# tsnb66/afivo-streamer

Hardware: AMD Instinct MI355X
Metric: cell-updates/s (fluid+MG V-cycle) (higher is better)
Workload: dtype f64; 1 GPU; s1-64; n_cell=64, leaf_cells=134217728, boxes=585, levels=4, coarse_solve=exact separable, fused_rhs=interior, face_field=from phi in the flux, vcycle_graphs=False, parallelism=single-gpu

## Files before the change

afivo-streamer_amd/csrc/afh_mg.hip:

```cpp
#include <hip/hip_ext.h>

#include <algorithm>
#include <cfloat>
#include <cmath>
#include <map>
#include <type_traits>

#include "afh_internal.h"
#include "afh_cs_direct.h"
#include "afh_pfmg_dev.h"

#include <mutex>

namespace afh {

struct Coef {
  double c[7];
};

constexpr int MAXMG = 16;
constexpr int CS_BOTTOM_SWEEPS = 16;
constexpr int CS_SMALL_CELLS = 4096;
constexpr int CS_DS_N = 16;
constexpr int CS_DS_CELLS = 1024;
// ... 866 lines not shown
__device__ __forceinline__ double apply7(const double *x, size_t c, size_t sj,
                                         size_t sk, const Coef &cf) {
  return cf.c[0] * x[c] + cf.c[1] * x[c - 1] + cf.c[2] * x[c + 1] +
         cf.c[3] * x[c - sj] + cf.c[4] * x[c + sj] + cf.c[5] * x[c - sk] +
         cf.c[6] * x[c + sk];
}

struct StConst {
  Coef cf;
  __device__ double apply(int, size_t, const double *x, size_t c, size_t sj, size_t sk) const {
    return apply7(x, c, sj, sk, cf);
  }
};

struct StVar {
  const double *const *vp, *const *bp;
  __device__ double apply(int id, size_t cv, const double *x, size_t c, size_t sj,
                          size_t sk) const {
    const double *v = vp[id - 1] + 7 * cv, *b = bp[id - 1];
    double a = v[0] * x[c] + v[1] * x[c - 1] + v[2] * x[c + 1] + v[3] * x[c - sj] +
               v[4] * x[c + sj] + v[5] * x[c - sk] + v[6] * x[c + sk];
    if (b) a = a - b[cv];
    return a;
  }
};

template <bool MAX, int K, bool GRAD = false>
__global__ void __launch_bounds__(256)
    k_residual(const double *__restrict__ phi, const double *__restrict__ rhs,
               double *__restrict__ tmp, const int32_t *__restrict__ ids,
               int nc, size_t bsz, Coef cf0, unsigned long long *red,
               const Coef *__restrict__ cft = nullptr,
               const afh_box_meta *__restrict__ meta = nullptr,
               double *__restrict__ nrm = nullptr, double gfac = 0.0) {
  const int t = blockIdx.x * blockDim.x + threadIdx.x;
  double mx = 0.0;
  if (t < nc * nc * (nc / K)) {
    const int id = ids[blockIdx.y];
    const Coef cf = cft ? cft[meta[id - 1].lvl - 1] : cf0;
    int i, j, kq;
    cell3(t, nc, i, j, kq);
    const int ng = nc + 2;
    const size_t sj = ng, sk = (size_t)ng * ng;
    const size_t o = (size_t)(id - 1) * bsz, c0 = ix3(ng, i, j, (kq - 1) * K + 1);
    const double *x = phi + o;
    double z[K + 2], xm[K], xp[K], ym[K], yp[K], r[K];
#pragma unroll
    for (int q = 0; q < K + 2; q++) z[q] = x[c0 + (q - 1) * sk];
#pragma unroll
    for (int q = 0; q < K; q++) {
      const size_t c = c0 + q * sk;
      xm[q] = x[c - 1];
      xp[q] = x[c + 1];
      ym[q] = x[c - sj];
      yp[q] = x[c + sj];
      r[q] = rhs[o + c];
    }
#pragma unroll
    for (int q = 0; q < K; q++) {
      const double a = cf.c[0] * z[q + 1] + cf.c[1] * xm[q] + cf.c[2] * xp[q] +
                       cf.c[3] * ym[q] + cf.c[4] * yp[q] + cf.c[5] * z[q] +
                       cf.c[6] * z[q + 2];
      const double v = r[q] - a;
      st_nt<AFH_NT_MG>(tmp + (o + c0 + q * sk), v);
      mx = fmax(mx, fabs(v));
    }
    if constexpr (GRAD) {
      const afh_box_meta &mb = meta[id - 1];
      const double gx = gfac / mb.dr[0], gy = gfac / mb.dr[1], gz = gfac / mb.dr[2];
#pragma unroll
      for (int q = 0; q < K; q++) {
        const double pv = z[q + 1];
        const double fxl = gx * (pv - xm[q]), fxh = gx * (xp[q] - pv);
        const double fyl = gy * (pv - ym[q]), fyh = gy * (yp[q] - pv);
        const double fzl = gz * (pv - z[q]), fzh = gz * (z[q + 2] - pv);
        const double a = fxl + fxh, b = fyl + fyh, c = fzl + fzh;
        st_nt<AFH_NT_MG>(nrm + (o + c0 + q * sk), 0.5 * sqrt(a * a + b * b + c * c));
      }
    }
  }
  if (MAX) block_max_to_shard(mx, red);
}

template <class St>
__global__ void k_rstr_fas(double *__restrict__ phi,
                           const double *__restrict__ rhs,
                           double *__restrict__ tmp,
                           const afh_box_meta *__restrict__ meta,
                           const int32_t *__restrict__ ids, int nc, size_t bsz,
                           St st) {
  const int hn = nc >> 1;
  const int t = blockIdx.x * blockDim.x + threadIdx.x;
  if (t >= hn * hn * hn) return;
  const int id = ids[blockIdx.y];
  const afh_box_meta &m = meta[id - 1];
  int i, j, k;
  cell3(t, hn, i, j, k);
  const int ng = nc + 2;
  const size_t sj = ng, sk = (size_t)ng * ng;
  const size_t o = (size_t)(id - 1) * bsz;
  const double *x = phi + o, *r = rhs + o;
  const int fi = 2 * i - 1, fj = 2 * j - 1, fk = 2 * k - 1;
  double sr = 0.0, sp = 0.0;
#pragma unroll
  for (int q = 0; q < 8; q++) {
    const int ci = fi + (q & 1), cj = fj + ((q >> 1) & 1), ck = fk + (q >> 2);
    const size_t c = ix3(ng, ci, cj, ck);
    const size_t cv = ((size_t)(ck - 1) * nc + (cj - 1)) * nc + (ci - 1);
    const double res = r[c] - st.apply(id, cv, x, c, sj, sk);
    if (q == 0) {
      sr = res;
      sp = x[c];
    } else {
      sr += res;
      sp += x[c];
    }
  }
  const size_t po = (size_t)(m.parent - 1) * bsz +
                    ix3(ng, ((m.ix[0] - 1) & 1) * hn + i,
                        ((m.ix[1] - 1) & 1) * hn + j,
                        ((m.ix[2] - 1) & 1) * hn + k);
  tmp[po] = 0.125 * sr;
  phi[po] = 0.125 * sp;
}

template <int K>
__global__ void __launch_bounds__(256)
    k_rstr_fas_col(double *__restrict__ phi, const double *__restrict__ rhs,
                   double *__restrict__ tmp, const afh_box_meta *__restrict__ meta,
                   const int32_t *__restrict__ ids, int nc, size_t bsz, Coef cf,
                   const double *__restrict__ fine) {
  const int hn = nc >> 1;
  const int t = blockIdx.x * blockDim.x + threadIdx.x;
  if (t >= hn * hn * (hn / K)) return;
  const int id = ids[blockIdx.y];
  const afh_box_meta &m = meta[id - 1];
  int i, j, kq;
  cell3(t, hn, i, j, kq);
  const int k0 = (kq - 1) * K + 1;
  const int ng = nc + 2;
  const size_t sj = ng;
  const size_t o = (size_t)(id - 1) * bsz;
  const double *x = fine + o, *r = rhs + o;
  const int fi = 2 * i - 1, fj = 2 * j - 1, f0 = 2 * k0 - 1;
  double c[2 * K + 2][4];
#pragma unroll
  for (int p = 0; p < 2 * K + 2; p++) {
    const size_t b = ix3(ng, fi, fj, f0 - 1 + p);
    c[p][0] = x[b];
    c[p][1] = x[b + 1];
    c[p][2] = x[b + sj];
    c[p][3] = x[b + sj + 1];
  }
  const size_t pb = (size_t)(m.parent - 1) * bsz;
  const int pi = ((m.ix[0] - 1) & 1) * hn + i, pj = ((m.ix[1] - 1) & 1) * hn + j,
            pk = ((m.ix[2] - 1) & 1) * hn;
#pragma unroll
  for (int q = 0; q < K; q++) {
    double sr = 0.0, sp = 0.0;
#pragma unroll
    for (int h = 0; h < 2; h++) {
      const int p = 2 * q + 1 + h;
      const size_t b = ix3(ng, fi, fj, f0 - 1 + p);
      const double xm0 = x[b - 1], xp0 = x[b + 2];
      const double xm1 = x[b + sj - 1], xp1 = x[b + sj + 2];
      const double ym0 = x[b - sj], ym1 = x[b - sj + 1];
// ... 241 lines not shown
    if (dd[3] < 1 && !later(3)) f[fx(1, i, j + 1, k)] = iy * (bc - pc) / dd[3];
    if (dd[4] < 1 && !later(4)) f[fx(2, i, j, k)] = iz * (pc - bc) / dd[4];
    if (dd[5] < 1 && !later(5)) f[fx(2, i, j, k + 1)] = iz * (bc - pc) / dd[5];
  }
}

__global__ void k_field_norm(const double *__restrict__ fcv,
                             double *__restrict__ nrm,
                             const int32_t *__restrict__ ids, int nc, size_t bsz,
                             size_t fsz) {
  const int t = blockIdx.x * blockDim.x + threadIdx.x;
  if (t >= nc * nc * nc) return;
  const int id = ids[blockIdx.y];
  int i, j, k;
  cell3(t, nc, i, j, k);
  const int nf = nc + 1;
  const size_t d3 = (size_t)nf * nf * nf;
  const double *f = fcv + (size_t)(id - 1) * fsz;
  const size_t fb = ((size_t)(k - 1) * nf + (j - 1)) * nf + (i - 1);
  const double a = f[fb] + f[fb + 1], b = f[d3 + fb] + f[d3 + fb + nf],
               cc = f[2 * d3 + fb] + f[2 * d3 + fb + (size_t)nf * nf];
  nrm[(size_t)(id - 1) * bsz + ix3(nc + 2, i, j, k)] = 0.5 * sqrt(a * a + b * b + cc * cc);
}

__global__ void k_corr_tmp(const double *__restrict__ phi,
                           double *__restrict__ tmp,
                           const int32_t *__restrict__ ids, size_t bsz) {
  const size_t t = (size_t)blockIdx.x * blockDim.x + threadIdx.x;
  if (t >= bsz) return;
  const size_t o = (size_t)(ids[blockIdx.y] - 1) * bsz + t;
  tmp[o] = phi[o] - tmp[o];
}

__global__ void k_box_copy(const double *__restrict__ src,
                           double *__restrict__ dst,
                           const int32_t *__restrict__ ids, size_t bsz) {
  const size_t t = (size_t)blockIdx.x * blockDim.x + threadIdx.x;
  if (t >= bsz) return;
  const size_t o = (size_t)(ids[blockIdx.y] - 1) * bsz + t;
  dst[o] = src ? src[o] : 0.0;
}

template <int K>
__global__ void __launch_bounds__(256)
    k_prolong(double *__restrict__ phi, const double *__restrict__ tmp,
              const afh_box_meta *__restrict__ meta,
              const int32_t *__restrict__ ids, int nc, size_t bsz) {
  const int t = blockIdx.x * blockDim.x + threadIdx.x;
  if (t >= nc * nc * (nc / K)) return;
  const int id = ids[blockIdx.y];
  const afh_box_meta &m = meta[id - 1];
  int i, j, kq;
  cell3(t, nc, i, j, kq);
  const int k0 = (kq - 1) * K + 1;
  const int ng = nc + 2, hn = nc >> 1;
  const size_t sk = (size_t)ng * ng;
  const int o0 = ((m.ix[0] - 1) & 1) * hn, o1 = ((m.ix[1] - 1) & 1) * hn,
            o2 = ((m.ix[2] - 1) & 1) * hn;
  const int i1 = o0 + ((i + 1) >> 1), i2 = i1 + 1 - 2 * (i & 1);
  const int j1 = o1 + ((j + 1) >> 1), j2 = j1 + 1 - 2 * (j & 1);
  const int P = o2 + ((k0 + 1) >> 1);
  const double *p = tmp + (size_t)(m.parent - 1) * bsz;
  const size_t c = (size_t)(id - 1) * bsz + ix3(ng, i, j, k0);
  double pv[K / 2 + 2][4], ph[K];
#pragma unroll
  for (int q = 0; q < K / 2 + 2; q++) {
    const size_t b = ix3(ng, 0, 0, P - 1 + q);
    pv[q][0] = p[b + (size_t)j1 * ng + i1];
    pv[q][1] = p[b + (size_t)j1 * ng + i2];
    pv[q][2] = p[b + (size_t)j2 * ng + i1];
    pv[q][3] = p[b + (size_t)j2 * ng + i2];
  }
#pragma unroll
  for (int q = 0; q < K; q++) ph[q] = phi[c + q * sk];
#pragma unroll
  for (int q = 0; q < K; q++) {
    const int a = (q & 1) ? (q + 1) / 2 : q / 2 + 1;
    const int b = (q & 1) ? (q + 3) / 2 : q / 2;
    st_nt<AFH_NT_MG>(phi + (c + q * sk),
                     ph[q] + (27 / 64.0) * pv[a][0] + (9 / 64.0) * pv[a][1] +
                         (9 / 64.0) * pv[a][2] + (3 / 64.0) * pv[a][3] +
                         (9 / 64.0) * pv[b][0] + (3 / 64.0) * pv[b][1] +
                         (3 / 64.0) * pv[b][2] + (1 / 64.0) * pv[b][3]);
  }
}

__global__ void k_gradient(const double *__restrict__ phi,
                           double *__restrict__ fcv, double *__restrict__ nrm,
                           const afh_box_meta *__restrict__ meta,
                           const int32_t *__restrict__ ids, int nc, size_t bsz,
                           size_t fsz, double fac) {
  const int t = blockIdx.x * blockDim.x + threadIdx.x;
  if (t >= nc * nc * nc) return;
  const int id = ids[blockIdx.y];
  const afh_box_meta &m = meta[id - 1];
  const int i = t % nc + 1, j = (t / nc) % nc + 1, k = t / (nc * nc) + 1;
  const int ng = nc + 2, nf = nc + 1;
  const double *p = phi + (size_t)(id - 1) * bsz;
  double *f = fcv ? fcv + (size_t)(id - 1) * fsz : nullptr;
  const size_t c = ix3(ng, i, j, k), sj = ng, sk = (size_t)ng * ng;
  const double ix_ = fac / m.dr[0], iy = fac / m.dr[1], iz = fac / m.dr[2];
  const double fxl = ix_ * (p[c] - p[c - 1]), fxh = ix_ * (p[c + 1] - p[c]);
  const double fyl = iy * (p[c] - p[c - sj]), fyh = iy * (p[c + sj] - p[c]);
  const double fzl = iz * (p[c] - p[c - sk]), fzh = iz * (p[c + sk] - p[c]);
  const size_t d3 = (size_t)nf * nf * nf;
  auto fx = [&](int d, int a, int b, int cc) {
    return (size_t)d * d3 + ((size_t)(cc - 1) * nf + (b - 1)) * nf + (a - 1);
  };
  if (fcv) {
    f[fx(0, i, j, k)] = fxl;
    if (i == nc) f[fx(0, nc + 1, j, k)] = fxh;
    f[fx(1, i, j, k)] = fyl;
    if (j == nc) f[fx(1, i, nc + 1, k)] = fyh;
    f[fx(2, i, j, k)] = fzl;
    if (k == nc) f[fx(2, i, j, nc + 1)] = fzh;
  }
  if (nrm) {
    const double a = fxl + fxh, b = fyl + fyh, cc = fzl + fzh;
    nrm[(size_t)(id - 1) * bsz + c] = 0.5 * sqrt(a * a + b * b + cc * cc);
  }
}

template <int NC, int K, bool NT = false, bool FC = true>
__global__ void __launch_bounds__(256)
    k_gradient_t(const double *__restrict__ phi, double *__restrict__ fcv,
                 double *__restrict__ nrm, const int32_t *__restrict__ ids,
                 size_t bsz, size_t fsz, const afh_box_meta *__restrict__ meta,
                 double fac) {
  constexpr int R = 256 / NC < NC ? 256 / NC : NC;
  constexpr int NG = NC + 2, NF = NC + 1;
  constexpr size_t SJ = NG, SK = (size_t)NG * NG, D3 = (size_t)NF * NF * NF;
  const Blk B = xcd_block();
  const int i = threadIdx.x % NC + 1;
  const int j = (B.x % (NC / R)) * R + threadIdx.x / NC + 1;
  const int k0 = (B.x / (NC / R)) * K + 1;
  const int id = ids[B.y];
  const double ix_ = fac / meta[id - 1].dr[0], iy = fac / meta[id - 1].dr[1],
               iz = fac / meta[id - 1].dr[2];
  const double *p = phi + (size_t)(id - 1) * bsz;
  double *f = fcv + (size_t)(id - 1) * fsz;
  double *nb = nrm ? nrm + (size_t)(id - 1) * bsz : nullptr;
  const size_t c0 = ((size_t)k0 * NG + j) * NG + i;
  double pc[K + 2], xm[K], xp[K], ym[K], yp[K];
#pragma unroll
  for (int q = 0; q < K + 2; q++) pc[q] = p[c0 + (q - 1) * SK];
#pragma unroll
  for (int q = 0; q < K; q++) {
    const size_t c = c0 + q * SK;
    xm[q] = p[c - 1];
    xp[q] = p[c + 1];
    ym[q] = p[c - SJ];
    yp[q] = p[c + SJ];
  }
#pragma unroll
  for (int q = 0; q < K; q++) {
    const int k = k0 + q;
    const double pv = pc[q + 1];
    const double fxl = ix_ * (pv - xm[q]), fxh = ix_ * (xp[q] - pv);
    const double fyl = iy * (pv - ym[q]), fyh = iy * (yp[q] - pv);
    const double fzl = iz * (pv - pc[q]), fzh = iz * (pc[q + 2] - pv);
    const size_t fb = ((size_t)(k - 1) * NF + (j - 1)) * NF + (i - 1);
    if (FC) {
      st_nt<NT>(f + fb, fxl);
      if (i == NC) st_nt<NT>(f + fb + 1, fxh);
      st_nt<NT>(f + D3 + fb, fyl);
      if (j == NC) st_nt<NT>(f + D3 + fb + NF, fyh);
// ... 731 lines not shown
    for (int nb = 0; nb < 6; nb++)
      if ((fm >> nb) & 1) rv = rv + b2r[(size_t)nb * L0.np + p] * B.bc[nb].value;
    if (vbc[q]) rv = rv + vbc[q][e];
    b[p] = rv;
    X0[p] = phi[c];
  }
  __syncthreads();
  PF_T(10);
  int cur = 0;
  const int iters = afh_pf::pf_solve_block(Lg, nl, wave_from, A, Aw, soff, Pw, X0, X1, b, r,
                                           &slot, tol, max_iter, &cur);
  const double *x = cur ? X1 : X0;
  for (int u = threadIdx.x; u < nid * n3; u += blockDim.x) {
    const int q = u / n3, e = u % n3, id = ids[q];
    const afh_box_meta &m = meta[id - 1];
    const int i = e % nc + 1, j = (e / nc) % nc + 1, k = e / (nc * nc) + 1;
    (void)q;
    const int p = (((m.ix[2] - 1) * nc + k - 1) * ny + (m.ix[1] - 1) * nc + j - 1) * nx +
                  (m.ix[0] - 1) * nc + i - 1;
    phi[(size_t)(id - 1) * bsz + ix3(nc + 2, i, j, k)] = x[p];
  }
  if (threadIdx.x == 0 && iters_out) *iters_out = iters;
#ifdef AFH_PFMG_TIMING
  PF_T(11);
  if (threadIdx.x == 0) {
    const unsigned long long *a = afh_pf::pf_tacc();
    printf("PFTIME nt %d np %d nl %d wave %d iters %d wall10ns %llu | relax %llu/%llu res %llu/%llu "
           "rstr %llu/%llu interp %llu/%llu dot %llu/%llu handoff %llu | wave relax %llu/%llu "
           "res %llu/%llu rstr %llu/%llu interp %llu/%llu | gather %llu scatter %llu\n",
           (int)blockDim.x, np, nl, wave_from, iters, wall_clock64() - w0, a[0], a[12], a[1],
           a[13], a[2], a[14], a[3], a[15], a[4], a[16], a[5], a[6], a[18], a[7], a[19], a[8],
           a[20], a[9], a[21], a[10], a[11]);
  }
#endif
}

}

using namespace afh;

#ifndef AFH_RES_K
#define AFH_RES_K 0
#endif
#ifndef AFH_RSTR_K
#define AFH_RSTR_K 4
#endif
struct afh_mg {
  afh_tree *t = nullptr;
  afh_mg_desc d;
  std::vector<Coef> lvl_c;
  CsParams P;
  int small_from = 0;
  size_t small_lds = 0;
  double *d_dtab = nullptr;
  std::vector<double> h_dtab;
  int tab_bc[6] = {0, 0, 0, 0, 0, 0};
  int fused_min = 0;
  bool force_tiles = false;
  bool rccl_capture = false;
  std::vector<char> rhs_halo;
  int vc_max_lvl = 0;
  bool grad_nt = true;
  uint64_t phi_gc_gen = UINT64_MAX;
  uint64_t phi_gc_meth = UINT64_MAX;
  int *cs_iters = nullptr;
  bool cs_direct_small = true;
  int cs_ds_cells = CS_DS_CELLS;
  bool pair_push = true;
  bool prolong_push = true;
  bool rstr_push = true;
  bool in_fmg = false;
  bool pair_xfetch = true;
  int tiles_min = 256;
  int *d_cycles = nullptr;
  int cycles_host = 0;
  bool cycles_on_dev = false;
  double *d_norm = nullptr;
  Coef *d_lvl_c = nullptr;
  std::vector<double> h_norm;
  bool rstr_col = true;
  int rstr_k = AFH_RSTR_K;
  int res_k = AFH_RES_K;
  int prolong_k = 4;
  int rstr_bs = 256;
  int wave_cells = CS_WAVE_CELLS;
  double *d_q[3] = {nullptr, nullptr, nullptr}, *d_qt[3] = {nullptr, nullptr, nullptr};
  double *d_e[3] = {nullptr, nullptr, nullptr};
  double *w1 = nullptr, *w2 = nullptr;
  int q_bc[6] = {0, 0, 0, 0, 0, 0};
  double *alt = nullptr;
  double *alt_priv = nullptr;
  std::vector<double *> h_vp, h_bp, h_dd, h_bv;
  std::vector<int32_t *> h_ix;
  std::vector<int> h_lsf_n;
  double **d_vp = nullptr, **d_bp = nullptr, **d_dd = nullptr, **d_bv = nullptr;
  int32_t **d_ix = nullptr;
  int *d_lsf_n = nullptr;
  int i_lsf = 0;
  bool var_dirty = false, any_var = false, any_lsf = false;
  struct Graph {
    hipGraphExec_t exec = nullptr;
    uint64_t meth_gen = 0;
    bool warm = false;
    std::vector<hipGraphExec_t> segs;
    std::vector<std::array<int32_t, 4>> ops;
    bool eager_only = false;
    void release() {
      if (exec) hipGraphExecDestroy(exec);
      for (hipGraphExec_t s : segs)
        if (s) hipGraphExecDestroy(s);
      exec = nullptr;
      segs.clear();
      ops.clear();
    }
  };
  std::map<int, Graph> graphs;
  bool use_graphs = true;
  bool seg_graphs = true;
  int64_t n_replays = 0, n_seg_replays = 0;
  std::vector<char> lvl_var;
  LevelList ids_c, ids_v, leaves_c, leaves_v, parents_c, parents_v, lsf_leaves;
  double *cs_old = nullptr;
  bool csd_on = true, csd_ok = false;
  std::vector<double> h_v1;
  int h_v1_id = 0;
  uint64_t v1_gen = 1, csd_v_gen = 0, csd_meth_gen = UINT64_MAX;
  double *d_csd_ainv = nullptr, *d_csd_g = nullptr;
  int grad_iv = 0;
  double grad_fac = -1.0;
  uint64_t grad_phi_gen = UINT64_MAX, grad_norm_gen = UINT64_MAX;
  std::map<int, std::vector<double>> h_vl1;
  std::vector<double> pf_a7;
  uint64_t pf_v1_gen = 0, pf_meth_gen = UINT64_MAX;
  int pf_nl = 0, pf_np = 0, pf_lds = 0, pf_wave = 0;
  bool pf_stage = false;
  PfLvl *d_pf_lvl = nullptr;
  double *d_pf_A = nullptr, *d_pf_P = nullptr, *d_pf_b2r = nullptr, *d_pf_x = nullptr;
  uint8_t *d_pf_fmask = nullptr;
  const double **d_pf_vbc = nullptr;
};

static int32_t build_table(afh_mg *mg) {
  const afh_bc *bc = mg->t->meth[mg->d.i_phi].bc;
  CsParams &P = mg->P;
  mg->h_dtab.assign((size_t)MAXMG * 64 * 2, 0.0);
  for (int m = 0; m < P.n_mg; m++)
    for (int c = 0; c < 64; c++) {
      double d = P.cdiag[m];
      for (int nb = 1; nb <= 6; nb++) {
        const int dd = (nb - 1) >> 1;
        const bool low = ((nb - 1) & 1) == 0;
        const int at = low ? (c >> (2 * dd)) & 1 : (c >> (2 * dd + 1)) & 1;
        if (!at || P.per[dd]) continue;
        if (bc[nb - 1].type == AFH_BC_DIRICHLET) d = d - P.hc[m][dd];
        else d = d + P.hc[m][dd];
      }
      mg->h_dtab[(m * 64 + c) * 2] = d;
      mg->h_dtab[(m * 64 + c) * 2 + 1] = 1 / d;
    }
  for (int q = 0; q < 6; q++) mg->tab_bc[q] = bc[q].type;
  AFH_HIP(hipStreamSynchronize(mg->t->stream));
  AFH_HIP(hipMemcpy(mg->d_dtab, mg->h_dtab.data(),
                    mg->h_dtab.size() * sizeof(double), hipMemcpyHostToDevice));
  P.dtab = mg->d_dtab;
  return AFH_OK;
}
// ... 100 lines not shown
  mg->h_ix.assign(t->nb, nullptr), mg->h_lsf_n.assign(t->nb, 0);
  mg->lvl_c.resize(t->nlvl);
  for (int l = 1; l <= t->nlvl; l++) {
    const double *dr = &t->lvl_dr[3 * (l - 1)];
    Coef &c = mg->lvl_c[l - 1];
    for (int q = 0; q < 3; q++) {
      double inv = 1 / (dr[q] * dr[q]);
      c.c[1 + 2 * q] = inv;
      c.c[2 + 2 * q] = inv;
    }
    double s = c.c[1];
    for (int q = 2; q < 7; q++) s = s + c.c[q];
    c.c[0] = -s - d->helmholtz_lambda;
  }
  AFH_HIP(hipMalloc(&mg->d_lvl_c, sizeof(Coef) * t->nlvl));
  AFH_HIP(hipMemcpy(mg->d_lvl_c, mg->lvl_c.data(), sizeof(Coef) * t->nlvl,
                    hipMemcpyHostToDevice));
  CsParams &P = mg->P;
  memset(&P, 0, sizeof P);
  int m = 0;
  for (int q = 0; q < 3; q++) {
    P.dims[0][q] = t->cgs[q];
    P.hc[0][q] = mg->lvl_c[0].c[1 + 2 * q];
  }
  P.cdiag[0] = mg->lvl_c[0].c[0];
  P.cmask = 63;
  for (int q = 0; q < 3; q++) {
    P.per[q] = t->periodic[q];
    if (P.per[q]) P.cmask &= ~(3 << (2 * q));
  }
  for (;;) {
    int *n = P.dims[m];
    bool ok = (n[0] % 2 == 0) && (n[1] % 2 == 0) && (n[2] % 2 == 0) &&
              n[0] >= 4 && n[1] >= 4 && n[2] >= 4 && m < MAXMG - 1;
    for (int q = 0; q < 3; q++) ok = ok && !(P.per[q] && (n[q] / 2) % 2 != 0);
    if (!ok) break;
    for (int q = 0; q < 3; q++) {
      P.dims[m + 1][q] = n[q] / 2;
      P.hc[m + 1][q] = 0.25 * P.hc[m][q];
    }
    const double *h = P.hc[m + 1];
    P.cdiag[m + 1] = -(h[0] + h[0] + h[1] + h[1] + h[2] + h[2]) -
                     d->helmholtz_lambda;
    m++;
  }
  P.n_mg = m + 1;
  mg->small_from = P.n_mg - 1;
  while (mg->small_from > 0) {
    const int *n = P.dims[mg->small_from - 1];
    if ((long)n[0] * n[1] * n[2] > CS_SMALL_CELLS) break;
    mg->small_from--;
  }
  mg->small_lds = 0;
  for (int q = 0; q < P.n_mg; q++) {
    P.halo[q] = 1;
    const int nx = P.dims[q][0], ny = P.dims[q][1];
    const bool p2 = nx > 0 && ny > 0 && (nx & (nx - 1)) == 0 && (ny & (ny - 1)) == 0;
    P.lg[q] = p2 ? (__builtin_ctz(nx) | (__builtin_ctz(ny) << 8)) : -1;
    if (q >= mg->small_from)
      mg->small_lds += 2 * sizeof(double) * (size_t)P.dims[q][0] * P.dims[q][1] *
                       P.dims[q][2];
  }
  if (mg->small_lds + sizeof(CsParams) + MAXMG * 128 * sizeof(double) > 160 * 1024)
    return set_error(AFH_ERR_UNSUPPORTED, "coarse-solver LDS levels too large");
  AFH_HIP(raise_dyn_lds((const void *)k_cs_small, (int)mg->small_lds));
  AFH_HIP(hipMalloc(&mg->d_dtab, (size_t)MAXMG * 64 * 2 * sizeof(double)));
  if (int32_t e = build_table(mg)) return e;
  if (const char *env = getenv("AFH_RCCL_CAPTURE")) mg->rccl_capture = atoi(env) != 0;
  if (const char *env = getenv("AFH_GSRB_FUSED_MIN_BOXES"))
    mg->fused_min = atoi(env);
  else if (fused_nc_ok(t->nc))
    mg->fused_min = t->nc >= 32 ? 64 : 1;
  if (const char *env = getenv("AFH_GSRB_TILES")) mg->force_tiles = atoi(env) != 0;
  if (const char *env = getenv("AFH_GRAPHS")) mg->use_graphs = atoi(env) != 0;
  if (const char *env = getenv("AFH_RSTR_COL")) mg->rstr_col = atoi(env) != 0;
  if (const char *env = getenv("AFH_RSTR_K")) {
    const int k = atoi(env);
    mg->rstr_k = k == 8 ? 8 : k == 4 ? 4 : 2;
  }
  if (const char *env = getenv("AFH_RES_K"))
    mg->res_k = atoi(env) == 8 ? 8 : atoi(env) == 2 ? 2 : 4;
  if (const char *env = getenv("AFH_PROLONG_K"))
    mg->prolong_k = atoi(env) == 8 ? 8 : atoi(env) == 2 ? 2 : 4;
  if (const char *env = getenv("AFH_CS_ELEC_DIRECT")) mg->csd_on = atoi(env) != 0;
  if (const char *env = getenv("AFH_CS_DIRECT_SMALL")) mg->cs_direct_small = atoi(env) != 0;
  if (const char *env = getenv("AFH_GSRB_TILES_MIN")) mg->tiles_min = atoi(env);
  if (const char *env = getenv("AFH_PAIR_XFETCH")) mg->pair_xfetch = atoi(env) != 0;
  if (const char *env = getenv("AFH_PAIR_PUSH")) mg->pair_push = atoi(env) != 0;
  if (const char *env = getenv("AFH_PROLONG_PUSH")) mg->prolong_push = atoi(env) != 0;
  if (const char *env = getenv("AFH_RSTR_PUSH")) mg->rstr_push = atoi(env) != 0;
  AFH_HIP(hipMalloc(&mg->cs_iters, sizeof(int)));
  AFH_HIP(hipMalloc(&mg->d_cycles, sizeof(int)));
  if (fused_nc_ok(t->nc) && mg->fused_min > 0) {
    bool any = false;
    for (int l = 2; l <= t->nlvl; l++) any |= t->lvl_total[l - 1] >= mg->fused_min;
    if (any) {
      if (!t->alt) {
        if (int32_t e2 = pool_alloc((void **)&t->alt_base,
                                    (size_t)t->nb * t->bsz * sizeof(double), "alt"))
          return e2;
        t->alt = t->alt_base;
        AFH_HIP(hipMemsetAsync(t->alt, 0, (size_t)t->nb * t->bsz * sizeof(double),
                               t->stream));
      }
      t->alt_refs++;
      mg->alt = t->alt;
    }
  }
  for (int q = 0; q < P.n_mg; q++) {
    size_t n = (size_t)(P.dims[q][0] + 2) * (P.dims[q][1] + 2) * (P.dims[q][2] + 2);
    AFH_HIP(hipMalloc(&P.u[q], n * sizeof(double)));
    AFH_HIP(hipMalloc(&P.f[q], n * sizeof(double)));
    AFH_HIP(hipMemsetAsync(P.u[q], 0, n * sizeof(double), t->stream));
    AFH_HIP(hipMemsetAsync(P.f[q], 0, n * sizeof(double), t->stream));
  }
  if (d->coarse_mode == AFH_COARSE_DIRECT) {
    const size_t n = (size_t)P.dims[0][0] * P.dims[0][1] * P.dims[0][2];
    for (int q = 0; q < 3; q++) {
      const size_t nd = P.dims[0][q];
      AFH_HIP(hipMalloc(&mg->d_q[q], nd * nd * sizeof(double)));
      AFH_HIP(hipMalloc(&mg->d_qt[q], nd * nd * sizeof(double)));
      AFH_HIP(hipMalloc(&mg->d_e[q], nd * sizeof(double)));
    }
    AFH_HIP(hipMalloc(&mg->w1, n * sizeof(double)));
    AFH_HIP(hipMalloc(&mg->w2, n * sizeof(double)));
    if (int32_t e = build_direct(mg)) return e;
  }
  AFH_HIP(hipStreamSynchronize(t->stream));
  *out = mg;
  return AFH_OK;
}

int32_t afh_mg_destroy(afh_mg *mg) {
  if (!mg) return AFH_OK;
  hipStreamSynchronize(mg->t->stream);
  for (auto &g : mg->graphs) g.second.release();
  for (int q = 0; q < mg->P.n_mg; q++) {
    hipFree(mg->P.u[q]);
    hipFree(mg->P.f[q]);
  }
  hipFree(mg->d_dtab);
  for (int q = 0; q < 3; q++) hipFree(mg->d_q[q]), hipFree(mg->d_qt[q]), hipFree(mg->d_e[q]);
  hipFree(mg->w1);
  hipFree(mg->w2);
  hipFree(mg->d_csd_ainv), hipFree(mg->d_csd_g);
  hipFree(mg->d_pf_lvl), hipFree(mg->d_pf_A), hipFree(mg->d_pf_P), hipFree(mg->d_pf_b2r);
  hipFree(mg->d_pf_x), hipFree(mg->d_pf_fmask), hipFree((void *)mg->d_pf_vbc);
  hipFree(mg->alt_priv);
  if (mg->alt && --mg->t->alt_refs == 0) {
    hipFree(mg->t->alt_base);
    mg->t->alt = mg->t->alt_base = nullptr;
  }
  for (auto *v : {&mg->h_vp, &mg->h_bp, &mg->h_dd, &mg->h_bv})
    for (double *q : *v) hipFree(q);
  for (int32_t *q : mg->h_ix) hipFree(q);
  hipFree(mg->d_vp), hipFree(mg->d_bp), hipFree(mg->d_dd), hipFree(mg->d_bv);
  hipFree(mg->d_ix), hipFree(mg->d_lsf_n), hipFree(mg->cs_old);
  hipFree(mg->cs_iters);
  hipFree(mg->d_cycles);
  hipFree(mg->d_norm);
  hipFree(mg->d_lvl_c);
  for (LevelList *L : {&mg->ids_c, &mg->ids_v, &mg->leaves_c, &mg->leaves_v,
                       &mg->parents_c, &mg->parents_v, &mg->lsf_leaves})
    hipFree(L->d);
  delete mg;
  return AFH_OK;
// ... 220 lines not shown

static bool rstr_push(const afh_mg *mg, int lvl, bool ghosts_valid) {
  const int nc = mg->t->nc;
  return ghosts_valid && mg->rstr_push && pair_push(mg) && !mg->any_var &&
         (nc == 4 || nc == 8 || nc == 16) && fused_level(mg, lvl - 1);
}

static int32_t update_coarse(afh_mg *mg, int lvl, bool ghosts_valid = false) {
  afh_tree *t = mg->t;
  const int nc = t->nc, hn = nc / 2;
  double *phi = t->ccv(mg->d.i_phi), *rhs = t->ccv(mg->d.i_rhs), *tmp = t->ccv(mg->d.i_tmp);
  if (rstr_push(mg, lvl, ghosts_valid)) {
    const GcArgs ga = t->gc_args(mg->d.i_phi);
    const int nid = t->ids.n(lvl), np = t->parents.n(lvl - 1);
    if (nid) {
      with_size<4, 8, 16>(nc, [&](auto NC_) {
        constexpr int NC = decltype(NC_)::value;
        hipLaunchKernelGGL(k_rstr_box<NC>, dim3(nid), dim3(NC >= 16 ? 512 : 64), 0, t->stream,
                           phi, rhs, tmp, t->d_boxes, t->ids.at(lvl), t->bsz,
                           mg->lvl_c[lvl - 1], ga);
      });
      AFH_LAUNCH_CHECK("k_rstr_box");
    }
    if (np) {
      with_bool(nc == 16, [&](auto big) {
        constexpr int NT = decltype(big)::value ? 512 : 256;
        hipLaunchKernelGGL(k_parent_rhs_box<NT>, dim3(np), dim3(NT), 0, t->stream, phi, rhs,
                           tmp, t->d_boxes, t->parents.at(lvl - 1), nc, t->bsz,
                           mg->lvl_c[lvl - 2]);
      });
      AFH_LAUNCH_CHECK("k_parent_rhs_box");
    }
    return AFH_OK;
  }
  const int RK = mg->rstr_k, BS = mg->rstr_bs;
  const int kc = !mg->rstr_col               ? 0
                 : RK == 8 && hn % 8 == 0    ? 8
                 : RK >= 4 && hn % 4 == 0    ? 4
                 : hn % 2 == 0               ? 2
                                             : 0;
  auto rstr = [&](const LevelList &L, auto st) -> int32_t {
    const int nid = L.n(lvl);
    if (!nid) return AFH_OK;
    bool col = false;
    if constexpr (!is_var<decltype(st)>)
      col = with_col(kc, [&](auto K_) {
        constexpr int K = decltype(K_)::value;
        hipLaunchKernelGGL(k_rstr_fas_col<K>, dim3((hn * hn * (hn / K) + BS - 1) / BS, nid),
                           dim3(BS), 0, t->stream, phi, rhs, tmp, t->d_boxes, L.at(lvl), nc,
                           t->bsz, st.cf, phi);
      });
    if (!col)
      hipLaunchKernelGGL(k_rstr_fas<decltype(st)>, dim3((hn * hn * hn + 255) / 256, nid),
                         dim3(256), 0, t->stream, phi, rhs, tmp, t->d_boxes, L.at(lvl), nc,
                         t->bsz, st);
    AFH_LAUNCH_CHECK(is_var<decltype(st)> ? "k_rstr_fas_v" : "k_rstr_fas");
    return AFH_OK;
  };
  int32_t e;
  if ((e = const_then_var(mg, lvl, t->ids, mg->ids_c, mg->ids_v, rstr))) return e;
  if ((e = call_hook(t, AFH_HOOK_RESTRICT, lvl, mg->d.i_phi)) ||
      (e = call_hook(t, AFH_HOOK_RESTRICT, lvl, mg->d.i_tmp)))
    return e;
  if ((e = gc_lvl(t, lvl - 1, mg->d.i_phi, 1, fused_level(mg, lvl - 1),
                  fused_level(mg, lvl - 1) ? 2 : 1)))
    return e;
  auto parent_rhs = [&](const LevelList &P, auto st) -> int32_t {
    const int np = P.n(lvl - 1);
    if (!np) return AFH_OK;
    hipLaunchKernelGGL(k_parent_rhs<decltype(st)>, dim3((unsigned)((t->bsz + 255) / 256), np),
                       dim3(256), 0, t->stream, phi, rhs, tmp, P.at(lvl - 1), nc, t->bsz, st);
    AFH_LAUNCH_CHECK(is_var<decltype(st)> ? "k_parent_rhs_v" : "k_parent_rhs");
    return AFH_OK;
  };
  return const_then_var(mg, lvl - 1, t->parents, mg->parents_c, mg->parents_v, parent_rhs);
}

static bool prolong_push(const afh_mg *mg, int lvl) {
  const int nc = mg->t->nc;
  return mg->prolong_push && pair_push(mg) && (nc == 4 || nc == 8 || nc == 16) &&
         fused_level(mg, lvl);
}

static int32_t correct_children(afh_mg *mg, int lvl) {
  afh_tree *t = mg->t;
  const int np = t->parents.n(lvl - 1), nc = t->nc;
  if (np) {
    hipLaunchKernelGGL(k_corr_tmp, dim3((unsigned)((t->bsz + 255) / 256), np),
                       dim3(256), 0, t->stream, t->ccv(mg->d.i_phi),
                       t->ccv(mg->d.i_tmp), t->parents.at(lvl - 1), t->bsz);
    AFH_LAUNCH_CHECK("k_corr_tmp");
  }
  const int nid = t->ids.n(lvl);
  if (nid && prolong_push(mg, lvl)) {
    const GcArgs ga = t->gc_args(mg->d.i_phi);
    with_size<4, 8, 16>(nc, [&](auto NC_) {
      constexpr int NC = decltype(NC_)::value;
      hipLaunchKernelGGL(k_prolong_box<NC>, dim3(nid), dim3(RbBox<NC>::NT), 0, t->stream,
                         t->ccv(mg->d.i_phi), t->ccv(mg->d.i_tmp), t->d_boxes, t->ids.at(lvl),
                         t->bsz, ga);
    });
    AFH_LAUNCH_CHECK("k_prolong_box");
  } else if (nid) {
    double *fphi = t->ccv(mg->d.i_phi);
    const int want = mg->prolong_k;
    const int K = want == 8 && nc % 8 == 0 ? 8 : want >= 4 && nc % 4 == 0 ? 4 : 2;
    const dim3 grid((nc * nc * (nc / K) + 255) / 256, nid);
    with_col(K, [&](auto K_) {
      hipLaunchKernelGGL(k_prolong<decltype(K_)::value>, grid, dim3(256), 0, t->stream, fphi,
                         t->ccv(mg->d.i_tmp), t->d_boxes, t->ids.at(lvl), nc, t->bsz);
    });
    AFH_LAUNCH_CHECK("k_prolong");
  }
  return AFH_OK;
}

extern "C++" {
template <int NC>
__global__ void __launch_bounds__(1024)
    k_cs_electrode(double *__restrict__ x, double *__restrict__ r,
                   const double *__restrict__ v, const double *__restrict__ b,
                   GcArgs ga, double dr0, double dr1, double dr2,
                   int *__restrict__ iters) {
  constexpr int NG = NC + 2, N3 = NC * NC * NC, G3 = NG * NG * NG;
  constexpr int SJ = NG, SK = NG * NG;
  __shared__ double X[G3], R[N3];
  __shared__ double s_d[16], s_m[16];
  const int tid = threadIdx.x, nt = blockDim.x;
  for (int e = tid; e < G3; e += nt) X[e] = x[e];
  for (int e = tid; e < N3; e += nt) {
    const int i = e % NC + 1, j = (e / NC) % NC + 1, k = e / (NC * NC) + 1;
    R[e] = r[ix3(NG, i, j, k)];
  }
  __syncthreads();
  constexpr int CPT = (N3 + 1023) / 1024;
  double old[CPT];
  int it;
  for (it = 1; it <= 200000; it++) {
#pragma unroll
    for (int q = 0; q < CPT; q++) {
      const int e = tid + q * nt;
      if (e < N3) {
        const int i = e % NC + 1, j = (e / NC) % NC + 1, k = e / (NC * NC) + 1;
        old[q] = X[ix3(NG, i, j, k)];
      }
    }
    for (int n = 1; n <= 2; n++) {
      for (int e = tid; e < N3; e += nt) {
        const int i = e % NC + 1, j = (e / NC) % NC + 1, k = e / (NC * NC) + 1;
        const int c = ix3(NG, i, j, k);
        const double *w = v + 7 * (size_t)e;
        double r1 = R[e];
        if (b) r1 = r1 + b[e];
        if (((i + j + k + n) & 1) == 0)
          X[c] = (r1 - w[1] * X[c - 1] - w[2] * X[c + 1] - w[3] * X[c - SJ] -
                  w[4] * X[c + SJ] - w[5] * X[c - SK] - w[6] * X[c + SK]) /
                 w[0];
        if (b) R[e] = r1 - b[e];
      }
      __syncthreads();
      for (int e = tid; e < 6 * NC * NC; e += nt) {
        const int nb = e / (NC * NC) + 1, ab = e % (NC * NC);
        const int d = (nb - 1) >> 1;
        const bool low = ((nb - 1) & 1) == 0;
        const int ta = d == 0 ? 1 : 0, tb = d == 2 ? 1 : 2;
        int p[3], q1[3];
        p[ta] = ab % NC + 1;
        p[tb] = ab / NC + 1;
        p[d] = low ? 0 : NC + 1;
        q1[0] = p[0], q1[1] = p[1], q1[2] = p[2];
        q1[d] = low ? 1 : NC;
        const afh_bc bc = ga.bc[nb - 1];
        const double drd = d == 0 ? dr0 : d == 1 ? dr1 : dr2;
        double c0, c1;
        switch (bc.type) {
        case AFH_BC_DIRICHLET: c0 = 2; c1 = -1; break;
        case AFH_BC_NEUMANN: c0 = drd * (low ? -1 : 1); c1 = 1; break;
        default: c0 = 1; c1 = 0; break;
        }
        X[ix3(NG, p[0], p[1], p[2])] = c0 * bc.value + c1 * X[ix3(NG, q1[0], q1[1], q1[2])];
      }
      __syncthreads();
    }
    double dm = 0.0, mm = 0.0;
#pragma unroll
    for (int q = 0; q < CPT; q++) {
      const int e = tid + q * nt;
      if (e < N3) {
        const int i = e % NC + 1, j = (e / NC) % NC + 1, k = e / (NC * NC) + 1;
        const double pv = X[ix3(NG, i, j, k)];
        dm = fmax(dm, fabs(pv - old[q]));
        mm = fmax(mm, fabs(pv));
      }
    }
    for (int o = 32; o > 0; o >>= 1) {
// ... 426 lines not shown
                               t->stream, P, m, n);
      }
      done = cyc + 1;
      if (tol) {
        double rr;
        if (int32_t e = norm2(1, rr)) return e;
        if (rr / bb < eps) break;
      }
    }
    AFH_LAUNCH_CHECK("coarse solver cycle");
    mg->cycles_host = done, mg->cycles_on_dev = false;
  }
  hipLaunchKernelGGL(k_cs_scatter, dim3((n3 + 255) / 256, nid), dim3(256), 0,
                     t->stream, P, t->ccv(mg->d.i_phi), t->d_boxes,
                     t->ids.at(1), nc, t->bsz);
  AFH_LAUNCH_CHECK("k_cs_scatter");
  return gc_lvl(t, 1, mg->d.i_phi, 1);
}

static int32_t box_copy(afh_tree *t, int lvl, const double *src, double *dst) {
  const int n = t->ids.n(lvl);
  if (!n) return AFH_OK;
  hipLaunchKernelGGL(k_box_copy, dim3((unsigned)((t->bsz + 255) / 256), n),
                     dim3(256), 0, t->stream, src, dst, t->ids.at(lvl), t->bsz);
  AFH_LAUNCH_CHECK("k_box_copy");
  return AFH_OK;
}

int32_t afh_mg_fas_fmg(afh_mg *mg, int32_t set_residual, int32_t have_guess) {
  if (!mg) return set_error(AFH_ERR_ARG, "null mg");
  afh_tree *t = mg->t;
  AFH_LIVE(t, "afh_mg_fas_fmg");
  if (int32_t ebc = phi_bc_check(mg)) return ebc;
  t->touch(mg->d.i_phi), t->touch(mg->d.i_rhs), t->touch(mg->d.i_tmp);
  const int nl = t->nlvl, i_phi = mg->d.i_phi;
  double *phi = t->ccv(i_phi), *tmp = t->ccv(mg->d.i_tmp);
  int32_t e;
  if ((e = prepare_all(mg))) return e;
  if (have_guess) {
    for (int lvl = nl; lvl >= 2; lvl--) {
      if (lvl == nl && (e = gc_lvl(t, lvl, i_phi, 1, fused_level(mg, lvl)))) return e;
      if ((e = update_coarse(mg, lvl))) return e;
    }
  } else {
    for (int lvl = nl; lvl >= 2; lvl--) {
      if ((e = box_copy(t, lvl, nullptr, phi)) ||
          (e = restrict_boxes(t, t->ids.at(lvl), t->ids.n(lvl), mg->d.i_rhs)) ||
          (e = call_hook(t, AFH_HOOK_RESTRICT, lvl, mg->d.i_rhs)))
        return e;
    }
  }
  if ((e = box_copy(t, 1, phi, tmp)) ||
      (e = afh_mg_fas_vcycle(mg, set_residual && nl == 1, 1)))
    return e;
  for (int lvl = 2; lvl <= nl; lvl++) {
    if ((e = box_copy(t, lvl, phi, tmp)) || (e = correct_children(mg, lvl)) ||
        (e = gc_lvl(t, lvl, i_phi, 1, fused_level(mg, lvl))))
      return e;
    mg->phi_gc_gen = t->gen[i_phi];
    mg->phi_gc_meth = t->meth_gen;
    mg->in_fmg = true;
    e = afh_mg_fas_vcycle(mg, set_residual && lvl == nl, lvl);
    mg->in_fmg = false;
    if (e) return e;
  }
  return AFH_OK;
}

}

static bool grad_fused(const afh_mg *mg, int max_lvl) {
  return mg->grad_iv > 0 && !mg->any_var && max_lvl == mg->t->nlvl;
}

static int32_t residual_levels(afh_mg *mg, int max_lvl, bool max_out) {
  afh_tree *t = mg->t;
  const int nc = t->nc, n3 = nc * nc * nc;
  auto *red = reinterpret_cast<unsigned long long *>(t->scratch) + 3 * RED_SHARDS;
  int32_t e;
  if (max_out && (e = red_init(t, 3, 0.0))) return e;
  const bool all_lvls = t->all_lvl_launch;
  const bool gr = grad_fused(mg, max_lvl);
  const int rk = mg->res_k ? mg->res_k : nc >= 32 ? 8 : 4;
  const int kc = nc % rk == 0 ? rk : nc % 4 == 0 ? 4 : 2;
  for (int lvl = 1; lvl <= max_lvl; lvl++) {
    for (int part = 0; part < 2; part++) {
      if (!max_out && part) break;
      const bool mx = max_out && !part;
      auto residual = [&](const LevelList &L, auto st) -> int32_t {
        using St = decltype(st);
        const int n_all = L.off[max_lvl] - L.off[0];
        const bool one = !is_var<St> && all_lvls && n_all <= 65535;
        const int n = one ? (lvl == 1 ? n_all : 0) : L.n(lvl);
        if (!n) return AFH_OK;
        double *phi = t->ccv(mg->d.i_phi), *rhs = t->ccv(mg->d.i_rhs), *tmp = t->ccv(mg->d.i_tmp);
        with_bool(mx, [&](auto MX) {
          if constexpr (is_var<St>)
            hipLaunchKernelGGL(k_residual_v<decltype(MX)::value>, dim3((n3 + 255) / 256, n),
                               dim3(256), 0, t->stream, phi, rhs, tmp, L.at(lvl), nc, t->bsz,
                               st, red);
          else
            with_bool(gr, [&](auto GR) {
              with_col(kc, [&](auto K) {
                hipLaunchKernelGGL(
                    (k_residual<decltype(MX)::value, decltype(K)::value, decltype(GR)::value>),
                    dim3((n3 / K + 255) / 256, n), dim3(256), 0, t->stream, phi, rhs, tmp,
                    L.at(lvl), nc, t->bsz, st.cf, red, one ? mg->d_lvl_c : nullptr,
                    (one || GR) ? t->d_boxes : nullptr, GR ? t->ccv(mg->grad_iv) : nullptr,
                    mg->grad_fac);
              });
            });
        });
        AFH_LAUNCH_CHECK(is_var<St> ? "k_residual_v" : "k_residual");
        return AFH_OK;
      };
      const LevelList *all[] = {&t->ids, &t->leaves, &t->parents},
                      *lc[] = {&mg->ids_c, &mg->leaves_c, &mg->parents_c},
                      *lv[] = {&mg->ids_v, &mg->leaves_v, &mg->parents_v};
      const int w = max_out ? 1 + part : 0;
      if ((e = const_then_var(mg, lvl, *all[w], *lc[w], *lv[w], residual))) return e;
    }
  }
  if (!max_out) return AFH_OK;
  return red_finish(t, 3, true);
}

static int32_t residual_fetch(afh_mg *mg, double *max_out) {
  return red_reduce_fetch(mg->t, 3, 1, 0, max_out, mg->d.i_tmp);
}

static int32_t vcycle_body(afh_mg *mg, int32_t set_residual, int max_lvl, bool max_out,
                           bool top_stale) {
  afh_tree *t = mg->t;
  int32_t e;
  mg->rhs_halo.assign(t->nlvl, 0);
  mg->vc_max_lvl = max_lvl;
  for (int lvl = max_lvl; lvl >= 2; lvl--) {
    if ((e = gsrb_boxes(mg, lvl, false, top_stale && lvl == max_lvl))) return e;
    if ((e = update_coarse(mg, lvl, !top_stale && (max_lvl == t->nlvl || mg->in_fmg) &&
                                        mg->phi_gc_meth == t->meth_gen)))
      return e;
  }
  if ((e = solve_coarse(mg))) return e;
  for (int lvl = 2; lvl <= max_lvl; lvl++) {
    if ((e = correct_children(mg, lvl))) return e;
    if (!prolong_push(mg, lvl) &&
        (e = gc_lvl_var(t, lvl, mg->d.i_phi, t->ccv(mg->d.i_phi),
                        t->gc_args(mg->d.i_phi), 1, fused_level(mg, lvl),
                        fused_level(mg, lvl) ? 2 : 1,
                        fused_level(mg, lvl) && pair_xfetch(mg) && mg->d.n_cycle_up >= 2 &&
                            !(mg->d.n_cycle_up & 1))))
      return e;
    if ((e = gsrb_boxes(mg, lvl, true))) return e;
  }
  if (set_residual) return residual_levels(mg, max_lvl, max_out);
  return AFH_OK;
}

static int32_t vcycle_segments(afh_mg *mg, afh_mg::Graph &g, int32_t set_residual,
                               int max_lvl, bool max_out, bool top_stale, bool &done) {
  afh_tree *t = mg->t;
  if (g.segs.empty()) {
    afh_tree::SegRec rec;
    AFH_HIP(hipStreamBeginCapture(t->stream, hipStreamCaptureModeThreadLocal));
    t->seg_rec = &rec;
    int32_t e = vcycle_body(mg, set_residual, max_lvl, max_out, top_stale);
    t->seg_rec = nullptr;
    hipGraph_t last = nullptr;
    const hipError_t ce = hipStreamEndCapture(t->stream, &last);
    if (ce == hipSuccess) rec.graphs.push_back(last);
    if (!e && ce != hipSuccess) e = set_error(AFH_ERR_DEVICE, "segment capture failed");
    for (size_t k = 0; k < rec.graphs.size() && !e; k++) {
      size_t nn = 0;
      hipGraphExec_t x = nullptr;
      if (hipGraphGetNodes(rec.graphs[k], nullptr, &nn) != hipSuccess ||
          (nn && hipGraphInstantiate(&x, rec.graphs[k], nullptr, nullptr, 0) != hipSuccess))
        e = set_error(AFH_ERR_DEVICE, "segment instantiation failed");
      g.segs.push_back(x);
    }
    for (hipGraph_t gr : rec.graphs)
      if (gr) hipGraphDestroy(gr);
    if (rec.bad) {
      g.release();
      g.eager_only = true;
      return AFH_OK;
    }
    if (e) {
      g.release();
      return e;
    }
    g.ops = rec.ops;
  }
  for (size_t k = 0; k < g.segs.size(); k++) {
    if (g.segs[k]) AFH_HIP(hipGraphLaunch(g.segs[k], t->stream));
    if (k < g.ops.size())
      if (int32_t e = call_hook(t, g.ops[k][0], g.ops[k][1], g.ops[k][2], nullptr, g.ops[k][3]))
// ... 353 lines not shown
```

Measured before the change: 12.34 billion cell-updates/s.

## Add flat paired-cell residual and prolongation kernels with 16-byte vector loads

Adds new residual and prolongation kernels in which each thread handles two adjacent x-cells across the full padded row. Loads and stores use 16-byte double2 accesses, and x-neighbours are exchanged through wavefront shuffles, with edge lanes fetching their halo directly. The goal is fewer memory transactions and less index arithmetic in these bandwidth-bound multigrid stages. The cost is threads wasted on ghost rows and columns, masked stores, and a change of the default residual column depth to 4. The new path applies only when arrays are 16-byte aligned and nc is at least 32.

```diff
diff --git a/afivo-streamer_amd/csrc/afh_mg.hip b/afivo-streamer_amd/csrc/afh_mg.hip
--- a/afivo-streamer_amd/csrc/afh_mg.hip
+++ b/afivo-streamer_amd/csrc/afh_mg.hip
@@ -972,6 +972,123 @@
   if (MAX) block_max_to_shard(mx, red);
 }
 
+typedef double dbl2 __attribute__((ext_vector_type(2)));
+
+__device__ __forceinline__ dbl2 ld2(const double *p) {
+  return *reinterpret_cast<const dbl2 *>(p);
+}
+
+template <bool NT>
+__device__ __forceinline__ void st_pair(double *p, double vx, double vy, bool sx, bool sy) {
+  if (sx && sy) {
+    const dbl2 v = {vx, vy};
+    if constexpr (NT) __builtin_nontemporal_store(v, reinterpret_cast<dbl2 *>(p));
+    else *reinterpret_cast<dbl2 *>(p) = v;
+  } else if (sx) {
+    st_nt<NT>(p, vx);
+  } else if (sy) {
+    st_nt<NT>(p + 1, vy);
+  }
+}
+
+struct FlatPair {
+  unsigned kq, p, j, m;
+  bool live;
+};
+__device__ __forceinline__ FlatPair flat_pair(int nc, int K) {
+  const unsigned hw = (nc + 2) >> 1, npp = hw * (nc + 2), total = npp * (nc / K);
+  const unsigned t0 = blockIdx.x * blockDim.x + threadIdx.x;
+  FlatPair f;
+  f.live = t0 < total;
+  const unsigned t = f.live ? t0 : total - 1;
+  f.kq = t / npp;
+  f.p = t - f.kq * npp;
+  f.j = f.p / hw;
+  f.m = f.p - f.j * hw;
+  return f;
+}
+
+template <bool MAX, int K, bool GRAD = false>
+__global__ void __launch_bounds__(256)
+    k_residual_flat(const double *__restrict__ phi, const double *__restrict__ rhs,
+                    double *__restrict__ tmp, const int32_t *__restrict__ ids, int nc,
+                    size_t bsz, Coef cf0, unsigned long long *red,
+                    const Coef *__restrict__ cft = nullptr,
+                    const afh_box_meta *__restrict__ meta = nullptr,
+                    double *__restrict__ nrm = nullptr, double gfac = 0.0) {
+  const FlatPair f = flat_pair(nc, K);
+  const int id = ids[blockIdx.y];
+  const Coef cf = cft ? cft[meta[id - 1].lvl - 1] : cf0;
+  const int ng = nc + 2;
+  const size_t sj = ng, sk = (size_t)ng * ng;
+  const size_t o = (size_t)(id - 1) * bsz, c0 = (size_t)(f.kq * K + 1) * sk + 2 * (size_t)f.p;
+  const double *x = phi + o;
+  const int lane = threadIdx.x & 63;
+  dbl2 z[K + 2], ym[K], yp[K], r[K];
+  double e[K];
+#pragma unroll
+  for (int q = 0; q < K + 2; q++) z[q] = ld2(x + (c0 + q * sk - sk));
+#pragma unroll
+  for (int q = 0; q < K; q++) {
+    const size_t c = c0 + q * sk;
+    ym[q] = ld2(x + (c - sj));
+    yp[q] = ld2(x + (c + sj));
+    r[q] = ld2(rhs + (o + c));
+  }
+  if (lane == 0 || lane == 63) {
+    const size_t ce = lane ? c0 + 2 : c0 - 1;
+#pragma unroll
+    for (int q = 0; q < K; q++) e[q] = x[ce + q * sk];
+  } else {
+#pragma unroll
+    for (int q = 0; q < K; q++) e[q] = 0.0;
+  }
+  const bool row = f.live && f.j >= 1 && f.j <= (unsigned)nc;
+  const bool sx = row && f.m >= 1, sy = row && f.m < (unsigned)(nc >> 1);
+  double xl[K], xr[K], mx = 0.0;
+#pragma unroll
+  for (int q = 0; q < K; q++) {
+    const double l = __shfl_up(z[q + 1].y, 1), h = __shfl_down(z[q + 1].x, 1);
+    xl[q] = lane == 0 ? e[q] : l;
+    xr[q] = lane == 63 ? e[q] : h;
+  }
+#pragma unroll
+  for (int q = 0; q < K; q++) {
+    const double ax = cf.c[0] * z[q + 1].x + cf.c[1] * xl[q] + cf.c[2] * z[q + 1].y +
+                      cf.c[3] * ym[q].x + cf.c[4] * yp[q].x + cf.c[5] * z[q].x +
+                      cf.c[6] * z[q + 2].x;
+    const double ay = cf.c[0] * z[q + 1].y + cf.c[1] * z[q + 1].x + cf.c[2] * xr[q] +
+                      cf.c[3] * ym[q].y + cf.c[4] * yp[q].y + cf.c[5] * z[q].y +
+                      cf.c[6] * z[q + 2].y;
+    const double vx = r[q].x - ax, vy = r[q].y - ay;
+    st_pair<AFH_NT_MG>(tmp + (o + c0 + q * sk), vx, vy, sx, sy);
+    if (sx) mx = fmax(mx, fabs(vx));
+    if (sy) mx = fmax(mx, fabs(vy));
+  }
+  if constexpr (GRAD) {
+    const afh_box_meta &mb = meta[id - 1];
+    const double gx = gfac / mb.dr[0], gy = gfac / mb.dr[1], gz = gfac / mb.dr[2];
+#pragma unroll
+    for (int q = 0; q < K; q++) {
+      double n2[2];
+#pragma unroll
+      for (int s = 0; s < 2; s++) {
+        const double pv = s ? z[q + 1].y : z[q + 1].x;
+        const double pxm = s ? z[q + 1].x : xl[q], pxp = s ? xr[q] : z[q + 1].y;
+        const double pym = s ? ym[q].y : ym[q].x, pyp = s ? yp[q].y : yp[q].x;
+        const double pzm = s ? z[q].y : z[q].x, pzp = s ? z[q + 2].y : z[q + 2].x;
+        const double fxl = gx * (pv - pxm), fxh = gx * (pxp - pv);
+        const double fyl = gy * (pv - pym), fyh = gy * (pyp - pv);
+        const double fzl = gz * (pv - pzm), fzh = gz * (pzp - pv);
+        const double a = fxl + fxh, b = fyl + fyh, c = fzl + fzh;
+        n2[s] = 0.5 * sqrt(a * a + b * b + c * c);
+      }
+      st_pair<AFH_NT_MG>(nrm + (o + c0 + q * sk), n2[0], n2[1], sx, sy);
+    }
+  }
+  if (MAX) block_max_to_shard(mx, red);
+}
+
 template <class St>
 __global__ void k_rstr_fas(double *__restrict__ phi,
                            const double *__restrict__ rhs,
@@ -1379,6 +1496,54 @@
                          (9 / 64.0) * pv[a][2] + (3 / 64.0) * pv[a][3] +
                          (9 / 64.0) * pv[b][0] + (3 / 64.0) * pv[b][1] +
                          (3 / 64.0) * pv[b][2] + (1 / 64.0) * pv[b][3]);
+  }
+}
+
+template <int K>
+__global__ void __launch_bounds__(256)
+    k_prolong_flat(double *__restrict__ phi, const double *__restrict__ tmp,
+                   const afh_box_meta *__restrict__ meta,
+                   const int32_t *__restrict__ ids, int nc, size_t bsz) {
+  const FlatPair f = flat_pair(nc, K);
+  const int id = ids[blockIdx.y];
+  const afh_box_meta &mb = meta[id - 1];
+  const int k0 = f.kq * K + 1;
+  const int ng = nc + 2, hn = nc >> 1, j = f.j;
+  const size_t sk = (size_t)ng * ng;
+  const int o0 = ((mb.ix[0] - 1) & 1) * hn, o1 = ((mb.ix[1] - 1) & 1) * hn,
+            o2 = ((mb.ix[2] - 1) & 1) * hn;
+  const int ia = o0 + f.m;
+  const int j1 = o1 + ((j + 1) >> 1), j2 = j1 + 1 - 2 * (j & 1);
+  const int P = o2 + ((k0 + 1) >> 1);
+  const double *p = tmp + (size_t)(mb.parent - 1) * bsz;
+  const size_t c = (size_t)(id - 1) * bsz + (size_t)k0 * sk + 2 * (size_t)f.p;
+  double pv[K / 2 + 2][4];
+  dbl2 ph[K];
+#pragma unroll
+  for (int q = 0; q < K / 2 + 2; q++) {
+    const size_t b = ix3(ng, 0, 0, P - 1 + q);
+    pv[q][0] = p[b + (size_t)j1 * ng + ia];
+    pv[q][1] = p[b + (size_t)j1 * ng + ia + 1];
+    pv[q][2] = p[b + (size_t)j2 * ng + ia];
+    pv[q][3] = p[b + (size_t)j2 * ng + ia + 1];
+  }
+#pragma unroll
+  for (int q = 0; q < K; q++) ph[q] = ld2(phi + (c + q * sk));
+  const bool row = f.live && j >= 1 && j <= nc;
+  const bool sx = row && f.m >= 1, sy = row && f.m < (unsigned)hn;
+#pragma unroll
+  for (int q = 0; q < K; q++) {
+    const int a = (q & 1) ? (q + 1) / 2 : q / 2 + 1;
+    const int b = (q & 1) ? (q + 3) / 2 : q / 2;
+    const double vx = ph[q].x + (27 / 64.0) * pv[a][0] + (9 / 64.0) * pv[a][1] +
+                      (9 / 64.0) * pv[a][2] + (3 / 64.0) * pv[a][3] +
+                      (9 / 64.0) * pv[b][0] + (3 / 64.0) * pv[b][1] +
+                      (3 / 64.0) * pv[b][2] + (1 / 64.0) * pv[b][3];
+    const double vy = ph[q].y + (27 / 64.0) * pv[a][1] + (9 / 64.0) * pv[a][0] +
+                      (9 / 64.0) * pv[a][3] + (3 / 64.0) * pv[a][2] +
+                      (9 / 64.0) * pv[b][1] + (3 / 64.0) * pv[b][0] +
+                      (3 / 64.0) * pv[b][3] + (1 / 64.0) * pv[b][2];
+    st_pair<AFH_NT_MG>(phi + (c + q * sk), vx, vy, sx, sy);
   }
 }
 
@@ -2276,6 +2441,7 @@
   int rstr_k = AFH_RSTR_K;
   int res_k = AFH_RES_K;
   int prolong_k = 4;
+  bool flat = true;
   int rstr_bs = 256;
   int wave_cells = CS_WAVE_CELLS;
   double *d_q[3] = {nullptr, nullptr, nullptr}, *d_qt[3] = {nullptr, nullptr, nullptr};
@@ -2542,6 +2708,7 @@
     mg->res_k = atoi(env) == 8 ? 8 : atoi(env) == 2 ? 2 : 4;
   if (const char *env = getenv("AFH_PROLONG_K"))
     mg->prolong_k = atoi(env) == 8 ? 8 : atoi(env) == 2 ? 2 : 4;
+  if (const char *env = getenv("AFH_MG_FLAT")) mg->flat = atoi(env) != 0;
   if (const char *env = getenv("AFH_CS_ELEC_DIRECT")) mg->csd_on = atoi(env) != 0;
   if (const char *env = getenv("AFH_CS_DIRECT_SMALL")) mg->cs_direct_small = atoi(env) != 0;
   if (const char *env = getenv("AFH_GSRB_TILES_MIN")) mg->tiles_min = atoi(env);
@@ -2928,6 +3095,18 @@
          fused_level(mg, lvl);
 }
 
+static bool mg_flat(const afh_mg *mg, int k, std::initializer_list<const void *> arrays) {
+  const int nc = mg->t->nc;
+  if (!mg->flat || nc < 32 || (nc & 1) || k < 4 || nc % k) return false;
+  for (const void *p : arrays)
+    if (reinterpret_cast<uintptr_t>(p) & 15) return false;
+  return true;
+}
+
+static unsigned flat_blocks(int nc, int k) {
+  return ((unsigned)((nc + 2) * (nc + 2) / 2 * (nc / k)) + 255) / 256;
+}
+
 static int32_t correct_children(afh_mg *mg, int lvl) {
   afh_tree *t = mg->t;
   const int np = t->parents.n(lvl - 1), nc = t->nc;
@@ -2951,12 +3130,20 @@
     double *fphi = t->ccv(mg->d.i_phi);
     const int want = mg->prolong_k;
     const int K = want == 8 && nc % 8 == 0 ? 8 : want >= 4 && nc % 4 == 0 ? 4 : 2;
-    const dim3 grid((nc * nc * (nc / K) + 255) / 256, nid);
+    const bool flat = mg_flat(mg, K, {fphi, t->ccv(mg->d.i_tmp)});
+    const dim3 grid(flat ? flat_blocks(nc, K) : (nc * nc * (nc / K) + 255) / 256, nid);
     with_col(K, [&](auto K_) {
-      hipLaunchKernelGGL(k_prolong<decltype(K_)::value>, grid, dim3(256), 0, t->stream, fphi,
+      constexpr int KC = decltype(K_)::value;
+      if constexpr (KC >= 4)
+        if (flat) {
+          hipLaunchKernelGGL(k_prolong_flat<KC>, grid, dim3(256), 0, t->stream, fphi,
+                             t->ccv(mg->d.i_tmp), t->d_boxes, t->ids.at(lvl), nc, t->bsz);
+          return;
+        }
+      hipLaunchKernelGGL(k_prolong<KC>, grid, dim3(256), 0, t->stream, fphi,
                          t->ccv(mg->d.i_tmp), t->d_boxes, t->ids.at(lvl), nc, t->bsz);
     });
-    AFH_LAUNCH_CHECK("k_prolong");
+    AFH_LAUNCH_CHECK(flat ? "k_prolong_flat" : "k_prolong");
   }
   return AFH_OK;
 }
@@ -3549,7 +3736,11 @@
   const bool all_lvls = t->all_lvl_launch;
   const bool gr = grad_fused(mg, max_lvl);
   const int rk = mg->res_k ? mg->res_k : nc >= 32 ? 8 : 4;
-  const int kc = nc % rk == 0 ? rk : nc % 4 == 0 ? 4 : 2;
+  int kc = nc % rk == 0 ? rk : nc % 4 == 0 ? 4 : 2;
+  const double *gnrm = gr ? t->ccv(mg->grad_iv) : nullptr;
+  const bool flat = mg_flat(mg, kc, {t->ccv(mg->d.i_phi), t->ccv(mg->d.i_rhs),
+                                     t->ccv(mg->d.i_tmp), gnrm});
+  if (flat && !mg->res_k) kc = 4;
   for (int lvl = 1; lvl <= max_lvl; lvl++) {
     for (int part = 0; part < 2; part++) {
       if (!max_out && part) break;
@@ -3569,16 +3760,26 @@
           else
             with_bool(gr, [&](auto GR) {
               with_col(kc, [&](auto K) {
+                constexpr int KC = decltype(K)::value;
+                const Coef *cft = one ? mg->d_lvl_c : nullptr;
+                const afh_box_meta *meta = (one || GR) ? t->d_boxes : nullptr;
+                double *nrm = GR ? t->ccv(mg->grad_iv) : nullptr;
+                if constexpr (KC >= 4)
+                  if (flat) {
+                    hipLaunchKernelGGL(
+                        (k_residual_flat<decltype(MX)::value, KC, decltype(GR)::value>),
+                        dim3(flat_blocks(nc, KC), n), dim3(256), 0, t->stream, phi, rhs, tmp,
+                        L.at(lvl), nc, t->bsz, st.cf, red, cft, meta, nrm, mg->grad_fac);
+                    return;
+                  }
                 hipLaunchKernelGGL(
-                    (k_residual<decltype(MX)::value, decltype(K)::value, decltype(GR)::value>),
+                    (k_residual<decltype(MX)::value, KC, decltype(GR)::value>),
                     dim3((n3 / K + 255) / 256, n), dim3(256), 0, t->stream, phi, rhs, tmp,
-                    L.at(lvl), nc, t->bsz, st.cf, red, one ? mg->d_lvl_c : nullptr,
-                    (one || GR) ? t->d_boxes : nullptr, GR ? t->ccv(mg->grad_iv) : nullptr,
-                    mg->grad_fac);
+                    L.at(lvl), nc, t->bsz, st.cf, red, cft, meta, nrm, mg->grad_fac);
               });
             });
         });
-        AFH_LAUNCH_CHECK(is_var<St> ? "k_residual_v" : "k_residual");
+        AFH_LAUNCH_CHECK(is_var<St> ? "k_residual_v" : flat ? "k_residual_flat" : "k_residual");
         return AFH_OK;
       };
       const LevelList *all[] = {&t->ids, &t->leaves, &t->parents},
```

Measured after the change: 12.61 billion cell-updates/s (median of 6 runs). 1.02x the previous value.
